# anands-repo/hello

Hardware: AMD Instinct MI355X
Metric: candidate sites/sec (whole node) (higher is better)
Workload: dtype f32

## Files before the change

### hello_amd/compiler.py

```python
from __future__ import annotations

from dataclasses import dataclass, field
from typing import Dict, List, Optional, Tuple

import numpy as np

from . import netspec as ns
from . import weights as wts

ROWS_READS0, ROWS_READS1, ROWS_ALLELES, ROWS_SITES = 0, 1, 2, 3
SEG_R0A, SEG_R1A, SEG_AS = 0, 1, 2
BUF_NONE, BUF_READS0, BUF_READS1, BUF_REF, BUF_FIRST_SCRATCH = -1, 0, 1, 2, 3
OP_XATTN_FRONT = 11
(OP_CONV1D, OP_MAXPOOL, OP_SEGSUM, OP_MIX, OP_HEAD, OP_CONCAT, OP_ADD, OP_READCONV_FUSED, OP_LAYERNORM,
 OP_COMPRESSOR_FUSED) = range(1, 11)
FLAG_RELU, FLAG_SRC_U8, FLAG_SOFTMAX, FLAG_MIX_REST, FLAG_SOFTPLUS, FLAG_WINOGRAD, FLAG_BF16X3, FLAG_BF16X3_32 = 1, 2, 4, 8, 16, 32, 64, 128
FLAG_LANE_SHIFT, MAX_LANES = 8, 8
OP_NAMES = {1: "conv1d", 2: "maxpool", 3: "segsum", 4: "mix", 5: "head", 6: "concat", 7: "add",
            8: "readconv_fused", 9: "layernorm", 10: "compressor_fused", 11: "xattn_front"}


@dataclass
class Value:
    vid: int
    domain: int
    length: int
    channels: int
    u8: bool = False

    @property
    def floats_per_row(self):
        return self.length * self.channels


@dataclass
class Op:
    kind: int
    domain: int
    src0: int = BUF_NONE
    src1: int = BUF_NONE
    dst: int = BUF_NONE
    res: int = BUF_NONE
    cin: int = 0
    cout: int = 0
    k: int = 0
    stride: int = 1
    pad: int = 0
    lin: int = 0
    lout: int = 0
# ... 498 lines not shown
        return n_experts, has_meta


def _fold_site_sums(ops: List[Op]) -> List[Op]:
    drop = set()
    for o in ops:
        if o.kind != OP_XATTN_FRONT or o.src1 == BUF_NONE:
            continue
        makers = [j for j, m in enumerate(ops) if m.kind == OP_SEGSUM and m.dst == o.src1]
        readers = [r for r in ops if r is not o and o.src1 in (r.src0, r.src1, r.res)]
        if len(makers) == 1 and not readers and ops[makers[0]].seg == SEG_AS and ops[makers[0]].src0 == o.src0:
            drop.add(makers[0])
            o.src1 = BUF_NONE
    return [o for j, o in enumerate(ops) if j not in drop]


def _fold_concats(ops: List[Op]) -> List[Op]:
    drop = set()
    for j, c in enumerate(ops):
        if c.kind != OP_CONCAT or c.cin % 16 or c.c1 % 16:
            continue
        readers = [r for r in ops if r is not c and c.dst in (r.src0, r.src1, r.res)]
        if len(readers) != 1:
            continue
        r = readers[0]
        if (r.kind == OP_CONV1D and r.src0 == c.dst and r.src1 == BUF_NONE and r.res == BUF_NONE and r.c1 <= 1
                and (r.flags & FLAG_WINOGRAD) and (r.flags & FLAG_RELU) and not (r.flags & (FLAG_BF16X3 | FLAG_SOFTPLUS))
                and r.cin == c.cin + c.c1):
            r.src0, r.src1, r.seg = c.src0, c.src1, c.cin
            drop.add(j)
    return [o for j, o in enumerate(ops) if j not in drop]


def assign_lanes(ops: List[Op], max_lanes: int = 4) -> int:
    producer: Dict[int, int] = {}
    lane_of: List[int] = []
    tail: Dict[int, int] = {}
    for i, o in enumerate(ops):
        front = o.kind == OP_XATTN_FRONT
        reads = [v for v in (o.src0, o.src1, BUF_NONE if front else o.res) if v >= 1000 and v in producer]
        pick = next((lane_of[producer[v]] for v in reads if tail.get(lane_of[producer[v]]) == producer[v]), None)
        if pick is None:
            unused = [lane for lane in range(max_lanes) if lane not in tail]
            pick = unused[0] if unused else (lane_of[producer[reads[0]]] if reads else 0)
        lane_of.append(pick)
        tail[pick] = i
        o.flags = (o.flags & ~(7 << FLAG_LANE_SHIFT)) | (pick << FLAG_LANE_SHIFT)
        if o.kind != OP_HEAD:
            producer[o.dst] = i
        if front:
            producer[o.res] = i
    return len(tail)


_SMALL_LAUNCH_US = {OP_READCONV_FUSED: 75.0, OP_COMPRESSOR_FUSED: 55.0, OP_XATTN_FRONT: 27.0, OP_CONV1D: 10.0, OP_HEAD: 8.0, OP_SEGSUM: 7.0}


def schedule_lanes(ops: List[Op]) -> List[Op]:
    shift = FLAG_LANE_SHIFT
    n = len(ops)
    producer: Dict[int, int] = {}
    preds: List[set] = [set() for _ in range(n)]
    last_on_lane: Dict[int, int] = {}
    for i, o in enumerate(ops):
        front = o.kind == OP_XATTN_FRONT
        for v in (o.src0, o.src1, BUF_NONE if front else o.res):
# ... 39 lines not shown
        if pool:
            fits = [p for p in pool if phys[p][1] >= need]
            pick = min(fits, key=lambda p: phys[p][1]) if fits else max(pool, key=lambda p: phys[p][1])
            pool.remove(pick)
            phys[pick] = (v.domain, max(phys[pick][1], need))
        else:
            pick = len(phys)
            phys.append((v.domain, need))
        assigned[vid] = pick

    for i, o in enumerate(ops):
        if o.kind == OP_XATTN_FRONT:
            place(o.dst)
            place(o.res)
            for vsrc in {o.src0, o.src1}:
                if reuse and vsrc >= 1000 and last_use.get(vsrc) == i and vsrc in assigned:
                    free[values[vsrc].domain].append(assigned[vsrc])
            continue
        if o.kind != OP_HEAD:
            place(o.dst)
        for vsrc in {o.src0, o.src1, o.res}:
            if reuse and vsrc >= 1000 and last_use.get(vsrc) == i and vsrc in assigned:
                free[values[vsrc].domain].append(assigned[vsrc])
    for o in ops:
        o.src0 = assigned.get(o.src0, o.src0)
        o.src1 = assigned.get(o.src1, o.src1)
        o.res = assigned.get(o.res, o.res)
        if o.kind != OP_HEAD:
            o.dst = assigned[o.dst]
    return phys


def compile_model(spec: ns.ModelSpec, state, fused: bool = True, winograd: bool = True, arithmetic: str = "fp32",
                  fold_site_sums: bool = True, lanes: bool = False) -> Program:
    low = _Lowering(spec, state, fused, winograd, arithmetic)
    n_experts, has_meta = low.lower()
    if arithmetic != "fp32" and not low.used_bf16x3:
        raise ValueError("arithmetic='bf16x3' / 'bf16x3+32' exists for the canonical 150 bp ReLU read convolver in the whole-kernel "
                         "Winograd form (fused=True, winograd=True): this model / these options do not run it")
    if fold_site_sums:
        low.ops = _fold_site_sums(low.ops)
        low.ops = _fold_concats(low.ops)
    n_lanes = assign_lanes(low.ops) if lanes else 1
    if n_lanes > 1:
        low.ops = schedule_lanes(low.ops)
    buffers = _allocate(low.ops, low.values, reuse=n_lanes == 1)
    return Program(
        spec_name=spec.name, window=spec.window, channels0=spec.channels[0],
        channels1=spec.channels[1] if spec.hybrid_inputs else 0,
        n_experts=n_experts, has_meta=has_meta, uses_ref=low.uses_ref, ops=low.ops,
        buffers=buffers, weights=low.blob.finish(), fused_read_convolver=low.used_fused,
        fused_compressor=low.used_fused_compressor, winograd=low.winograd, arithmetic=arithmetic, n_lanes=n_lanes)
```

### hello_amd/csrc/engine.hip

```cpp
#include <hip/hip_runtime.h>

#include <cstdarg>
#include <cstdio>
#include <cstring>
#include <new>
#include <stdexcept>
#include <string>
#include <vector>

#include "../../include/hello_mi355x.h"
#include "kernels.h"

namespace {

thread_local std::string g_last_error;

int fail(int code, const char* fmt, ...) {
    char buf[512];
    va_list ap;
    va_start(ap, fmt);
    vsnprintf(buf, sizeof(buf), fmt, ap);
    va_end(ap);
    g_last_error = buf;
    return code;
// ... 63 lines not shown
        if (bytes <= cap) return 0;
        if (p) (void)hipHostFree(p);
        p = nullptr;
        size_t want = bytes + bytes / 8 + 256;
        if (hipHostMalloc(&p, want, hipHostMallocDefault) != hipSuccess) return -1;
        cap = want;
        return 0;
    }
    void release() {
        if (p) (void)hipHostFree(p);
        p = nullptr;
        cap = 0;
    }
};

}

struct hello_engine {
    int device = 0;
    hello_model_desc desc{};
    std::vector<hello_op> ops;
    std::vector<hello_buffer> buffers;
    float* d_weights = nullptr;
    size_t n_weight_floats = 0;

    std::vector<DevBuf> scratch;
    DevBuf d_csr;
    PinnedBuf h_csr;
    DevBuf d_logits, d_meta, d_post, d_rcl0, d_rcl1;
    DevBuf d_out_small;
    PinnedBuf h_io;
    std::vector<DevBuf> d_partial;
    std::vector<int> partial_of;
    int n_lanes = 1;
    std::vector<hipStream_t> lane_streams;
    std::vector<hipEvent_t> op_done;
    std::vector<std::vector<int>> op_waits;
    std::vector<int> lane_tail;
    hipEvent_t ev_lanes_go = nullptr;
    DevBuf d_feat_in, d_feat_out;
    DevBuf d_support;
    hipStream_t own_stream = nullptr;
    hipStream_t last_stream = nullptr;
    hipEvent_t ev_staged = nullptr;
    hipEvent_t ev_start = nullptr, ev_stop = nullptr;
    bool staged_pending = false;
    bool timed = false;
    bool profiling = false;
    std::vector<std::vector<hipEvent_t>> prof_events;
    int prof_count = 0;
    int prof_filter = 0;
    int debug_op = -1;
    DevBuf d_debug;
    size_t debug_floats = 0;
    int stamp_mode = 0;
    DevBuf d_stamps;
    int32_t stamp_layout[5] = {0, 0, 0, 0, 0};

    int32_t *roff0 = nullptr, *roff1 = nullptr, *aoff = nullptr, *site_of_allele = nullptr;
    int32_t *allele_of_read0 = nullptr, *allele_of_read1 = nullptr;
    int32_t *group_slot0 = nullptr, *group_slot1 = nullptr, *slot_off0 = nullptr, *slot_off1 = nullptr;
    hello::ReadConvPlan plan0{1, 0, 0}, plan1{1, 0, 0};
    bool wide_trunk[2] = {false, false};
    int64_t* pair_off = nullptr;
};

// ... 249 lines not shown
    const int n_ops = d->n_ops;
    auto lane_of = [&](int i) { return lane_of_op(d->ops[i]); };
    for (int i = 0; i < n_ops; ++i) plan.n_lanes = lane_of(i) + 1 > plan.n_lanes ? lane_of(i) + 1 : plan.n_lanes;
    if (plan.n_lanes == 1) return 0;
    std::vector<int> writer(d->n_buffers, -1);
    plan.op_waits.assign(n_ops, {});
    plan.lane_tail.assign(plan.n_lanes, -1);
    plan.read_elsewhere.assign(n_ops, 0);
    for (int i = 0; i < n_ops; ++i) {
        const hello_op& o = d->ops[i];
        const bool front = o.kind == HELLO_OP_XATTN_FRONT;
        const int reads[3] = {o.src0, o.src1, front ? HELLO_BUF_NONE : o.res};
        for (int b : reads) {
            if (b < HELLO_BUF_FIRST_SCRATCH) continue;
            const int w = writer[b];
            if (w < 0) return fail(HELLO_ERR_MODEL, "laned program: op %d reads buffer %d before any op wrote it", i, b);
            if (lane_of(w) != lane_of(i)) {
                plan.op_waits[i].push_back(w);
                plan.read_elsewhere[w] = 1;
            }
        }
        const int writes[2] = {o.kind == HELLO_OP_HEAD ? HELLO_BUF_NONE : o.dst, front ? o.res : HELLO_BUF_NONE};
        for (int b : writes) {
            if (b < HELLO_BUF_FIRST_SCRATCH) continue;
            if (writer[b] >= 0)
                return fail(HELLO_ERR_MODEL, "laned program: ops %d and %d both write buffer %d (a program with lanes may not reuse buffers)", writer[b], i, b);
            writer[b] = i;
        }
        plan.lane_tail[lane_of(i)] = i;
    }
    return 0;
}

template <typename T>
T* carve(char*& cursor, size_t count) {
    T* p = reinterpret_cast<T*>(cursor);
    cursor += (count * sizeof(T) + 15) & ~size_t(15);
    return p;
}

}

extern "C" {

const char* hello_last_error(void) { return g_last_error.c_str(); }
int hello_abi_version(void) { return HELLO_ABI_VERSION; }

int hello_engine_create(const hello_model_desc* desc, const void* folded_weights, size_t nbytes,
                        int hip_device, hello_engine** out) try {
    if (!out) return fail(HELLO_ERR_ARG, "out is NULL");
    *out = nullptr;
    if (int rc = validate_model(desc)) return rc;
    LanePlan lanes;
    if (int rc = analyse_lanes(desc, lanes)) return rc;
    if (!folded_weights || nbytes == 0 || (nbytes % 4)) return fail(HELLO_ERR_ARG, "bad weight blob");
    int n_dev = 0;
    if (hipGetDeviceCount(&n_dev) != hipSuccess || n_dev <= 0)
        return fail(HELLO_ERR_NOGPU, "no HIP device visible: the HIP engine cannot run");
    if (hip_device < 0 || hip_device >= n_dev) return fail(HELLO_ERR_ARG, "device %d out of range", hip_device);
    hipDeviceProp_t prop;
    HIP_TRY(hipGetDeviceProperties(&prop, hip_device));
    if (strncmp(prop.gcnArchName, "gfx950", 6) != 0)
        return fail(HELLO_ERR_NOGPU, "device %d is %s; this engine is built for gfx950 only", hip_device,
                    prop.gcnArchName);
    HIP_TRY(hipSetDevice(hip_device));

    hello_engine* e = new hello_engine();
    e->device = hip_device;
    e->desc = *desc;
    e->ops.assign(desc->ops, desc->ops + desc->n_ops);
    e->buffers.assign(desc->buffers, desc->buffers + desc->n_buffers);
    e->desc.ops = e->ops.data();
    e->desc.buffers = e->buffers.data();
    e->n_weight_floats = nbytes / 4;
    for (const hello_op& o : e->ops) {
        size_t w_end = 0, b_end = 0;
        if (o.kind == HELLO_OP_CONV1D) {
            const bool wino = (o.flags & HELLO_FLAG_WINOGRAD) != 0;
            const size_t cpad = wino ? (size_t)o.cout : (size_t)((o.cout + 31) / 32) * 32;
            const int cing = o.cin / (o.c1 > 1 ? o.c1 : 1);
            const size_t kpad = wino ? (size_t)(hello::conv1d_wino_outputs_per_tile(o.lin) + 2) * cing
                                     : (size_t)((o.k * cing + 31) / 32) * 32;
            w_end = (size_t)o.w_off + cpad * kpad;
            b_end = (size_t)o.b_off + cpad;
        } else if (o.kind == HELLO_OP_HEAD) {
            w_end = (size_t)o.w_off + (size_t)o.cout * o.cin;
            b_end = (size_t)o.b_off + o.cout;
        } else if (o.kind == HELLO_OP_LAYERNORM) {
            w_end = (size_t)o.w_off + o.cin;
            b_end = (size_t)o.b_off + o.cin;
        } else if (o.kind == HELLO_OP_COMPRESSOR_FUSED) {
            w_end = (size_t)o.w_off + hello::compressor_weight_floats(o.k);
            b_end = (size_t)o.b_off;
        } else if (o.kind == HELLO_OP_XATTN_FRONT) {
            w_end = (size_t)o.w_off + hello::xattn_front_weight_floats();
            b_end = (size_t)o.b_off;
        } else if (o.kind == HELLO_OP_READCONV_FUSED) {
            w_end = (size_t)o.w_off + (o.cout == 128 ? hello::readconv_wide_weight_floats()
                                                     : hello::readconv_weight_floats(o.k, (o.flags & HELLO_FLAG_WINOGRAD) != 0, desc->window));
            b_end = (size_t)o.b_off;
            if (o.cout == 128) e->wide_trunk[o.seg == HELLO_SEG_READS1_TO_ALLELES ? 1 : 0] = true;
        }
        if (w_end > e->n_weight_floats || b_end > e->n_weight_floats) {
            delete e;
            return fail(HELLO_ERR_MODEL, "a weight block runs past the end of the blob");
        }
    }
// ... 439 lines not shown
            if (e->partial_of[i] >= 0)
                if (int rc = ensure(e->d_partial[e->partial_of[i]], slots * hello::readconv_frame_rows(d.window) * frame_ch * sizeof(float))) return rc;
    }
    if (d.n_experts == 3) HIP_TRY(hipMemsetAsync(d_logits, 0, logit_bytes, stream));

    auto ptr = [&](int id) -> void* {
        if (id == HELLO_BUF_NONE) return nullptr;
        if (id < HELLO_BUF_FIRST_SCRATCH) return const_cast<void*>(buf_ptr[id]);
        return e->scratch[id].p;
    };

    HIP_TRY(hipEventRecord(e->ev_start, stream));
    int op_index = 0;
    std::vector<hipEvent_t>* ring = nullptr;
    if (e->profiling && e->prof_count < (int)e->prof_events.size() &&
        e->prof_events[e->prof_count].size() == e->ops.size() + 1)
        ring = &e->prof_events[e->prof_count];
    auto mark = [&](int slot) -> int {
        hipEvent_t& ev = (*ring)[slot];
        if (!ev) HIP_TRY(hipEventCreate(&ev));
        HIP_TRY(hipEventRecord(ev, stream));
        return 0;
    };
    const int n_ops_total = (int)e->ops.size();
    auto wanted = [&](int i) { return i >= 0 && i < n_ops_total && (!e->prof_filter || e->ops[i].kind == e->prof_filter); };
    const bool laned = e->n_lanes > 1;
    if (laned) {
        if (ring || e->debug_op >= 0 || (e->stamp_mode & 1))
            return fail(HELLO_ERR_ARG, "per-op profiling / debug capture / stamps need the sequential program (this engine runs lanes)");
        HIP_TRY(hipEventRecord(e->ev_lanes_go, stream));
        for (int l = 1; l < e->n_lanes; ++l) HIP_TRY(hipStreamWaitEvent(e->lane_streams[l], e->ev_lanes_go, 0));
    }
    hipStream_t const call_stream = stream;
    for (const hello_op& o : e->ops) {
        const int lane = laned ? (o.flags & HELLO_FLAG_LANE_MASK) >> HELLO_FLAG_LANE_SHIFT : 0;
        hipStream_t const stream = lane ? e->lane_streams[lane] : call_stream;
        if (laned)
            for (int w : e->op_waits[op_index]) HIP_TRY(hipStreamWaitEvent(stream, e->op_done[w], 0));
        if (ring && (wanted(op_index) || wanted(op_index - 1)))
            if (int rc = mark(op_index)) return rc;
        const long long rows = rows_of(o.domain, S, A, R0, R1);
        switch (o.kind) {
            case HELLO_OP_CONV1D: {
                hello::ConvArgs a{};
                a.src = ptr(o.src0);
                a.dst = (float*)ptr(o.dst);
                a.res = (const float*)ptr(o.res);
                a.w = e->d_weights + o.w_off;
                a.bias = e->d_weights + o.b_off;
                a.m_total = rows * o.lout;
                a.groups = o.c1 > 1 ? o.c1 : 1;
                a.src2 = o.src1 != HELLO_BUF_NONE ? (const float*)ptr(o.src1) : nullptr;
                a.split = o.src1 != HELLO_BUF_NONE ? o.seg : 0;
                a.lin = o.lin; a.lout = o.lout; a.cin = o.cin / a.groups; a.cin_stride = o.cin; a.cout = o.cout;
                a.k = o.k; a.stride = o.stride; a.pad = o.pad;
                a.kpad = ((o.k * a.cin + 31) / 32) * 32;
                a.cout_pad = ((o.cout + 31) / 32) * 32;
                a.relu = (o.flags & HELLO_FLAG_RELU) ? 1 : ((o.flags & HELLO_FLAG_SOFTPLUS) ? 2 : 0);
                a.src_u8 = (o.flags & HELLO_FLAG_SRC_U8) ? 1 : 0;
                a.wino = (o.flags & HELLO_FLAG_WINOGRAD) ? 1 : 0;
                if (!a.src) return fail(HELLO_ERR_ARG, "op %d reads an input the caller did not supply", op_index);
                if (a.wino) {
                    a.kpad = (hello::conv1d_wino_outputs_per_tile(o.lin) + 2) * a.cin;
                    a.cout_pad = o.cout;
                    if (!hello::conv1d_wino_supported(a))
                        return fail(HELLO_ERR_MODEL, "op %d: this convolution has no Winograd form", op_index);
// ... 14 lines not shown
                                             o.lin * o.cin, stream));
                break;
            }
            case HELLO_OP_MIX:
                HIP_TRY(hello::launch_mix((const float*)ptr(o.src0), (const float*)ptr(o.src1), (float*)ptr(o.dst),
                                          e->site_of_allele, rows, o.lin * o.cin, o.a0, o.a1,
                                          (o.flags & HELLO_FLAG_MIX_REST) != 0, stream));
                break;
            case HELLO_OP_HEAD: {
                float* outp;
                long long so, sr;
                if (o.dst == 3) { outp = d_meta; so = 1; sr = 3; }
                else { outp = d_logits + (long long)o.dst * A; so = 0; sr = 1; }
                HIP_TRY(hello::launch_head((const float*)ptr(o.src0), e->d_weights + o.w_off, e->d_weights + o.b_off,
                                           outp, rows, o.lin, o.cin, o.cout, so, sr,
                                           (o.flags & HELLO_FLAG_SOFTMAX) ? 1 : 0, stream));
                break;
            }
            case HELLO_OP_CONCAT:
                HIP_TRY(hello::launch_concat((const float*)ptr(o.src0), (const float*)ptr(o.src1), (float*)ptr(o.dst),
                                             rows * o.lin, o.cin, o.c1, stream));
                break;
            case HELLO_OP_ADD:
                HIP_TRY(hello::launch_add((const float*)ptr(o.src0), (const float*)ptr(o.src1), (float*)ptr(o.dst),
                                          rows * o.lin * o.cin, stream));
                break;
            case HELLO_OP_COMPRESSOR_FUSED: {
                hello::CompressorArgs a{};
                a.frames = (const float*)ptr(o.src0);
                a.dst = (float*)ptr(o.dst);
                a.w = e->d_weights + o.w_off;
                a.n_items = rows;
                a.blocks = o.k;
                HIP_TRY(hello::launch_compressor_fused(a, stream));
                break;
            }
            case HELLO_OP_XATTN_FRONT: {
                hello::XattnFrontArgs a{};
                a.alleles = (const float*)ptr(o.src0);
                a.sites = o.src1 == HELLO_BUF_NONE ? nullptr : (const float*)ptr(o.src1);
                a.owner = e->site_of_allele;
                a.site_off = e->aoff;
                a.y2 = (float*)ptr(o.dst);
                a.sc = (float*)ptr(o.res);
                a.w = e->d_weights + o.w_off;
                a.n_items = rows;
                a.a0 = o.a0;
                a.a1 = o.a1;
                a.rest = (o.flags & HELLO_FLAG_MIX_REST) ? 1 : 0;
                HIP_TRY(hello::launch_xattn_front(a, stream));
                break;
            }
            case HELLO_OP_LAYERNORM:
                HIP_TRY(hello::launch_layernorm((const float*)ptr(o.src0), (const float*)ptr(o.res), (float*)ptr(o.dst),
                                                e->d_weights + o.w_off, e->d_weights + o.b_off, rows * o.lin, o.cin, o.a0,
                                                (o.flags & HELLO_FLAG_RELU) ? 1 : ((o.flags & HELLO_FLAG_SOFTPLUS) ? 2 : 0), stream));
                break;
            case HELLO_OP_READCONV_FUSED: {
                const bool t1 = o.seg == HELLO_SEG_READS1_TO_ALLELES;
                hello::ReadConvArgs a{};
                if (o.flags & HELLO_FLAG_SRC_U8) {
                    a.reads = (const uint8_t*)ptr(o.src0);
                    a.channels = o.cin;
                } else {
                    a.pooled = (const float*)ptr(o.src0);
                }
// ... 23 lines not shown
                    const int stamp_waves = hello::readconv_stamp_waves();
                    if ((e->stamp_mode & 1) && !t1 && total > 0) {
                        if (wide || !a.reads) return fail(HELLO_ERR_ARG, "stamps: the canonical fused read convolver from the bytes only");
                        const long long wgs = plan.rest_wgs ? plan.bulk_wgs + plan.rest_wgs : (long long)((total + (long long)G * plan.groups_per_wg - 1) / ((long long)G * plan.groups_per_wg));
                        const int slots = hello::readconv_stamp_slots();
                        const size_t bytes = (size_t)wgs * stamp_waves * plan.groups_per_wg * slots * sizeof(uint64_t);
                        if (bytes > e->d_stamps.cap) {
                            HIP_TRY(hipStreamSynchronize(stream));
                            if (e->d_stamps.ensure(bytes)) return fail(HELLO_ERR_HIP, "device allocation of %zu bytes failed", bytes);
                        }
                        HIP_TRY(hipMemsetAsync(e->d_stamps.p, 0, bytes, stream));
                        a.stamps = (unsigned long long*)e->d_stamps.p;
                        a.stamp_groups = plan.groups_per_wg;
                        a.stamp_mode = e->stamp_mode;
                        const int32_t lay[5] = {(int32_t)wgs, stamp_waves, plan.groups_per_wg, slots, (int32_t)(plan.rest_wgs ? plan.bulk_wgs : wgs)};
                        for (int i = 0; i < 5; ++i) stamp_lay[i] = lay[i];
                        e->stamp_layout[0] = 0;
                    }
                    HIP_TRY(wide ? hello::launch_readconv_wide(a, stream) : hello::launch_readconv_fused(a, stream));
                    if (plan.rest_wgs) {
                        hello::ReadConvArgs b = a;
                        if (b.stamps) b.stamps += (size_t)plan.bulk_wgs * stamp_waves * plan.groups_per_wg * hello::readconv_stamp_slots();
                        if (b.reads) b.reads += bulk_reads * d.window * o.cin;
                        else b.pooled += bulk_reads * (long long)o.lin * o.cin;
                        b.allele_of_read += bulk_reads;
                        b.slot_of_group += plan.bulk_wgs;
                        b.groups_per_wg = 1;
                        b.n_reads = total - bulk_reads;
                        HIP_TRY(wide ? hello::launch_readconv_wide(b, stream) : hello::launch_readconv_fused(b, stream));
                    }
                    if (a.stamps)
                        for (int i = 0; i < 5; ++i) e->stamp_layout[i] = stamp_lay[i];
                }
                HIP_TRY(hello::launch_readconv_finalize((const float*)e->d_partial[e->partial_of[op_index]].p, t1 ? e->slot_off1 : e->slot_off0,
                                                        (float*)ptr(o.dst), A, o.lout, o.cout, stream));
                break;
            }
        }
        if (op_index == e->debug_op) {
            const size_t per_row = o.kind == HELLO_OP_CONCAT ? (size_t)o.lout * (o.cin + o.c1)
                                   : (o.kind == HELLO_OP_CONV1D || o.kind == HELLO_OP_READCONV_FUSED || o.kind == HELLO_OP_COMPRESSOR_FUSED || o.kind == HELLO_OP_XATTN_FRONT) ? (size_t)o.lout * o.cout
                                   : (o.kind == HELLO_OP_MAXPOOL ? (size_t)o.lout * o.cin : (size_t)o.lin * o.cin);
            const size_t n = (size_t)rows * per_row;
            if (n * sizeof(float) > e->d_debug.cap) {
                HIP_TRY(hipStreamSynchronize(stream));
                if (e->d_debug.ensure(n * sizeof(float))) return fail(HELLO_ERR_HIP, "device allocation of %zu bytes failed", n * sizeof(float));
            }
            HIP_TRY(hipMemcpyAsync(e->d_debug.p, ptr(o.dst), n * sizeof(float), hipMemcpyDeviceToDevice, stream));
            e->debug_floats = n;
        }
        if (laned && e->op_done[op_index]) HIP_TRY(hipEventRecord(e->op_done[op_index], stream));
        ++op_index;
    }
    if (laned)
        for (int l = 1; l < e->n_lanes; ++l)
            if (e->lane_tail[l] >= 0) HIP_TRY(hipStreamWaitEvent(stream, e->op_done[e->lane_tail[l]], 0));
    if (ring) {
        if (int rc = mark(op_index)) return rc;
        e->prof_count++;
    }
    if (posteriors)
        HIP_TRY(hello::launch_posteriors(d_logits, d.n_experts == 3 ? d_meta : nullptr, e->aoff, e->pair_off, S, A,
                                         d.n_experts, n_pairs, d_post, stream));
    HIP_TRY(hipEventRecord(e->ev_stop, stream));
    e->timed = true;

    char* const h_out = out_total_small ? (char*)e->h_io.p + SMALL_IO : nullptr;
    if (out_total_small) {
// ... 227 lines not shown
```

### hello_amd/csrc/kernels.h

```cpp
#pragma once
#include <hip/hip_runtime.h>
#include <stdint.h>

namespace hello {

int device_cus();

struct ConvArgs {
    const void* src;
    const float* src2;
    int split;
    float* dst;
    const float* res;
    const float* w;
    const float* bias;
    long long m_total;
    int lin, lout, cin, cout, k, stride, pad;
    int cin_stride;
    int groups;
    int kpad;
    int cout_pad;
    int relu;
    int src_u8;
    unsigned wino_rows;
// ... 46 lines not shown
    int winograd;
    int window;
    int softplus;
    int bf16x3;
    unsigned long long* stamps;
    int stamp_groups;
    int stamp_mode;
};
int readconv_stamp_slots();
int readconv_stamp_waves();
bool readconv_supports_window(int window);
int readconv_reads_per_group(int window);
int readconv_frame_rows(int window);
int readconv_groups_per_workgroup(long long n_reads, int window);
struct ReadConvPlan {
    int groups_per_wg;
    long long bulk_wgs;
    long long rest_wgs;
};
ReadConvPlan readconv_plan(long long n_reads, int window);
ReadConvPlan readconv_wide_plan(long long n_reads);
int readconv_weight_floats(int extra_blocks, bool winograd, int window);
int readconv_bf16x3_extra_floats(int extra_blocks);
bool readconv_supports_extra_blocks(int extra_blocks);
hipError_t launch_readconv_fused(const ReadConvArgs& a, hipStream_t stream);
hipError_t launch_readconv_finalize(const float* partial, const int32_t* slot_off, float* frames, int n_alleles,
                                    int frame_rows, int channels, hipStream_t stream);
int readconv_wide_weight_floats();
int readconv_wide_reads_per_group();
hipError_t launch_readconv_wide(const ReadConvArgs& a, hipStream_t stream);

struct CompressorArgs {
    const float* frames;
    float* dst;
    const float* w;
    long long n_items;
    int blocks;
    int items_per_wg;
};
int small_launch_items_per_wg(long long n_items, int most);
int compressor_weight_floats(int blocks);
bool compressor_supports_blocks(int blocks);
hipError_t launch_compressor_fused(const CompressorArgs& a, hipStream_t stream);

struct XattnFrontArgs {
    const float* alleles;
    const float* sites;
    const int32_t* owner;
    const int32_t* site_off;
    float* y2;
    float* sc;
    const float* w;
    long long n_items;
    float a0, a1;
    int rest;
    int items_per_wg;
};
int xattn_front_weight_floats();
hipError_t launch_xattn_front(const XattnFrontArgs& a, hipStream_t stream);

struct FeaturizeArgs {
    const uint8_t* bases;
    const uint8_t* quals;
    const long long* read_off;
    const uint32_t* cigars;
    const long long* cigar_off;
// ... 28 lines not shown
```

### hello_amd/csrc/readconv_fused.hip

```cpp
#include <cstdlib>
#include <type_traits>

#include "kernels.h"

namespace hello {

typedef float f32x4 __attribute__((ext_vector_type(4)));

namespace rc {

constexpr int S1_STEPS = 6;
template <bool WINO, bool F33 = false>
struct Offs {
    static constexpr int KT = WINO ? 4 : 3;
    static constexpr int W3232 = 2 * KT * 2 * 256, W3264 = 4 * 3 * 2 * 256, W3264S = 4 * 1 * 2 * 256;
    static constexpr int W6464 = 4 * KT * 4 * 256;
    static constexpr int W6464D = F33 ? 4 * 5 * 4 * 256 : W6464;
    static constexpr int W3232D = F33 ? 2 * 5 * 2 * 256 : W3232;
    static constexpr int OFF_B = 0;
    static constexpr int OFF_C1 = OFF_B + 6 * (W3232D + 32);
    static constexpr int OFF_SC = OFF_C1 + W3264 + 64;
    static constexpr int OFF_C2 = OFF_SC + W3264S + 64;
    static constexpr int OFF_D = OFF_C2 + W6464D + 64;
    static constexpr int W_TRUNK = OFF_D + 6 * (W6464D + 64);
// ... 1567 lines not shown
    static constexpr int THREADS = 64 * NW;
    static constexpr int L0 = 36, L1 = 18;
    static constexpr int NSREG = 3 * (L1 * G / 48);
    static constexpr int BUF_FLOATS = rc::cmax((L0 * G + 2) * 64, (L1 * G + 2) * 128);
    static constexpr int LDS_BYTES = 2 * BUF_FLOATS * 4 + 64;
    static constexpr int W11 = 4 * 1 * 4 * 256, WS = 8 * 3 * 4 * 256, WSC = 8 * 1 * 4 * 256, WB = 8 * 8 * 5 * 256;
    static constexpr int OFF_11 = 0, OFF_S = OFF_11 + W11 + 64, OFF_SC = OFF_S + WS + 128, OFF_B = OFF_SC + WSC + 128;
    static constexpr int off_conv(int i) { return OFF_B + i * (WB + 128); }
    static constexpr int total(int blocks) { return off_conv(1 + 2 * blocks); }
};
}

int compressor_weight_floats(int blocks) { return cc::Cfg::total(blocks); }
bool compressor_supports_blocks(int blocks) { return blocks >= 2 && blocks <= 4; }

template <int NB>
__global__ __launch_bounds__(cc::Cfg::THREADS, 2) void compressor_kernel(CompressorArgs a) {
    using CF = cc::Cfg;
    constexpr int G = CF::G, L0 = CF::L0, L1 = CF::L1;
    extern __shared__ __attribute__((aligned(16))) float smem[];
    float* const bufA = smem;
    float* const bufB = smem + CF::BUF_FLOATS;
    float* const dump = smem + 2 * CF::BUF_FLOATS;
    const int tid = threadIdx.x, lane = tid & 63;
    const int wave = __builtin_amdgcn_readfirstlane(tid >> 6);
    const long long item0 = (long long)blockIdx.x * a.items_per_wg;
    const int n_here = (int)((a.n_items - item0) < a.items_per_wg ? (a.n_items - item0) : a.items_per_wg);
    const float* __restrict__ W = a.w;
    const f32x4 zero4 = {0.f, 0.f, 0.f, 0.f};

    f32x4 w11[4];
    load_weights<4>(w11, W + CF::OFF_11, wave % 4, lane);
    {
        const f32x4* src = (const f32x4*)(a.frames + item0 * (L0 * 64));
        constexpr int NLD = G * L0 * 16 / CF::THREADS;
        static_assert(NLD * CF::THREADS == G * L0 * 16, "the input image divides evenly over the threads");
        f32x4 v[NLD];
#pragma unroll
        for (int k = 0; k < NLD; ++k) {
            const int f = tid + CF::THREADS * k;
            v[k] = (f / (L0 * 16)) < n_here ? src[f] : zero4;
        }
#pragma unroll
        for (int k = 0; k < NLD; ++k) {
            const int f = tid + CF::THREADS * k;
            *(f32x4*)(bufA + img_off<64, SW_OLD>(1 + (f >> 4), f & 15)) = v[k];
        }
        if (tid < 16) ((f32x4*)bufA)[tid] = zero4;
        else if (tid < 32) ((f32x4*)bufB)[tid - 16] = zero4;
    }
    __syncthreads();
    f32x4 sreg[CF::NSREG];
    const bool full = n_here == G;
    const int live0 = (n_here * L0 + 15) / 16, live1 = (n_here * L1 + 15) / 16;
    if (full)
        conv_layer<CF, 64, 64, 1, 1, 0, L0, L0, L0, L0 * G / 16, MODE_PLAIN, false, GEOM_TRUNK, 16, L0 * G, false, SW_OLD, SW_W>(
            bufA, bufB, w11, nullptr, W + CF::OFF_11 + CF::W11, sreg, 0u, dump, wave, lane);
    else
        conv_layer<CF, 64, 64, 1, 1, 0, L0, L0, L0, L0 * G / 16, MODE_PLAIN, false, GEOM_TRUNK, 16, L0 * G, false, SW_OLD, SW_W, true>(
            bufA, bufB, w11, nullptr, W + CF::OFF_11 + CF::W11, sreg, 0u, dump, wave, lane, 0, (live0 - wave / 4 + 1) / 2);
    f32x4 ws[12], wsc[4];
    load_weights<12>(ws, W + CF::OFF_S, wave, lane);
    load_weights<4>(wsc, W + CF::OFF_SC, wave, lane);
    __syncthreads();
    if (tid < 64) ((f32x4*)bufA)[(tid & 31) + (tid >> 5) * (L1 * G + 1) * 32] = zero4;
    if (full)
        conv_layer<CF, 64, 128, 3, 2, 1, L0, L1, L1, L1 * G / 16, MODE_PLAIN, false, GEOM_TRUNK, 16, L1 * G, true, SW_W, SW_3>(
            bufB, bufA, ws, nullptr, W + CF::OFF_S + CF::WS, sreg, 0u, dump, wave, lane);
    else
        conv_layer<CF, 64, 128, 3, 2, 1, L0, L1, L1, L1 * G / 16, MODE_PLAIN, false, GEOM_TRUNK, 16, L1 * G, true, SW_W, SW_3, true>(
            bufB, bufA, ws, nullptr, W + CF::OFF_S + CF::WS, sreg, 0u, dump, wave, lane, 0, live1);
    conv_layer<CF, 64, 128, 1, 2, 0, L0, L1, L1, CF::NSREG, MODE_TO_REGS, false, GEOM_WTRIPLE, 16, L1 * G, false, SW_W, SW_3>(
        bufB, nullptr, wsc, nullptr, W + CF::OFF_SC + CF::WSC, sreg, 0u, dump, wave, lane);
    f32x4 w3[2][5];
// ... 16 lines not shown
        __syncthreads();
        static_for<0, NB>([&](auto bc) {
            constexpr int blk = decltype(bc)::value;
            constexpr int off_a = CF::off_conv(1 + 2 * blk), off_b = CF::off_conv(2 + 2 * blk);
            wino3_layer<CF, 128, MODE_PLAIN, false, L1, SW_3, true, PARTIAL>(bufB, bufA, w3, slice(off_a), slice(off_b),
                                                                            W + off_a + CF::WB, wave, lane, live_tiles);
            __syncthreads();
            if constexpr (blk < NB - 1)
                wino3_layer<CF, 128, MODE_RESID_INPLACE, false, L1, SW_3, true, PARTIAL>(
                    bufA, bufB, w3, slice(off_b), slice(CF::off_conv(3 + 2 * blk)), W + off_b + CF::WB, wave, lane, live_tiles);
            else
                wino3_layer<CF, 128, MODE_RESID_INPLACE, true, L1, SW_3, true, PARTIAL>(bufA, bufB, w3, slice(off_b), nullptr,
                                                                                       W + off_b + CF::WB, wave, lane, live_tiles);
            __syncthreads();
        });
    };
    if (live_tiles == L1 * G / 48) f33_layers(std::false_type{});
    else f33_layers(std::true_type{});
    f32x4* dst = (f32x4*)(a.dst + item0 * (L1 * 128));
    for (int f = tid; f < n_here * L1 * 32; f += CF::THREADS)
        dst[f] = *(const f32x4*)(bufB + img_off<128, SW_3>(1 + (f >> 5), f & 31));
}

int small_launch_items_per_wg(long long n_items, int most) {
    const long long cus = device_cus();
    const long long n = (n_items + cus - 1) / cus;
    return (int)(n < 1 ? 1 : (n <= 2 ? n : most));
}

hipError_t launch_compressor_fused(const CompressorArgs& args, hipStream_t stream) {
    if (args.n_items <= 0) return hipSuccess;
    CompressorArgs a = args;
    if (a.items_per_wg == 0) a.items_per_wg = small_launch_items_per_wg(a.n_items, cc::Cfg::G);
    if (!compressor_supports_blocks(a.blocks) || !a.frames || !a.dst || !a.w || a.items_per_wg < 1 || a.items_per_wg > cc::Cfg::G) return hipErrorInvalidValue;
    static bool configured_on[64] = {};
    int dev = 0;
    if (hipGetDevice(&dev) != hipSuccess || dev < 0 || dev >= 64) return hipErrorInvalidDevice;
    if (!configured_on[dev]) {
        hipError_t e = hipFuncSetAttribute((const void*)compressor_kernel<2>, hipFuncAttributeMaxDynamicSharedMemorySize, cc::Cfg::LDS_BYTES);
        if (e == hipSuccess)
            e = hipFuncSetAttribute((const void*)compressor_kernel<3>, hipFuncAttributeMaxDynamicSharedMemorySize, cc::Cfg::LDS_BYTES);
        if (e == hipSuccess)
            e = hipFuncSetAttribute((const void*)compressor_kernel<4>, hipFuncAttributeMaxDynamicSharedMemorySize, cc::Cfg::LDS_BYTES);
        if (e != hipSuccess) return e;
        configured_on[dev] = true;
    }
    const unsigned grid = (unsigned)((a.n_items + a.items_per_wg - 1) / a.items_per_wg);
    if (a.blocks == 2) hipLaunchKernelGGL(compressor_kernel<2>, dim3(grid), dim3(cc::Cfg::THREADS), cc::Cfg::LDS_BYTES, stream, a);
    else if (a.blocks == 3) hipLaunchKernelGGL(compressor_kernel<3>, dim3(grid), dim3(cc::Cfg::THREADS), cc::Cfg::LDS_BYTES, stream, a);
    else hipLaunchKernelGGL(compressor_kernel<4>, dim3(grid), dim3(cc::Cfg::THREADS), cc::Cfg::LDS_BYTES, stream, a);
    return hipGetLastError();
}


namespace xf {
struct Cfg {
    static constexpr int ACT = rc::ACT_RELU;
    static __device__ __forceinline__ float act(float x) { return fmaxf(x, 0.f); }
    static constexpr int G = 8, NW = 8, THREADS = 64 * NW;
    static constexpr int L = 18, LO = 9;
    static constexpr int NSREG = 1;
    static constexpr int A_FLOATS = (L * G + 2) * 128;
    static constexpr int B_ROWS = 2 * (16 * 5) + 2;
    static constexpr int LDS_BYTES = (A_FLOATS + B_ROWS * 128) * 4 + 64;
    static constexpr int W11 = 8 * 1 * 8 * 256, WS = 16 * 3 * 8 * 256, WSC = 16 * 1 * 8 * 256;
    static constexpr int OFF_11 = 0, OFF_S = OFF_11 + W11 + 128, OFF_SC = OFF_S + WS + 256, TOTAL = OFF_SC + WSC + 256;
};
// ... 492 lines not shown
```

### hello_amd/engine.py

```python
from __future__ import annotations

import ctypes as C
import logging
import os
from typing import Optional, Sequence, Tuple

import numpy as np

from . import compiler
from . import netspec as ns

_log = logging.getLogger(__name__)

_LIB_PATH = os.environ.get("HELLO_LIB") or os.path.join(os.path.dirname(os.path.abspath(__file__)),
                                                        "libhello_mi355x.so")
HELLO_IN_DEVICE, HELLO_OUT_DEVICE, HELLO_LAYOUT_RCL = 1, 2, 4
ABI_VERSION = 2
LANES_MAX_SITES = 64

class HelloOp(C.Structure):
    _fields_ = [("kind", C.c_int32), ("domain", C.c_int32), ("src0", C.c_int32), ("src1", C.c_int32),
                ("dst", C.c_int32), ("res", C.c_int32), ("cin", C.c_int32), ("cout", C.c_int32),
                ("k", C.c_int32), ("stride", C.c_int32), ("pad", C.c_int32), ("lin", C.c_int32),
                ("lout", C.c_int32), ("flags", C.c_int32), ("seg", C.c_int32), ("c1", C.c_int32),
# ... 68 lines not shown


def _is_torch(x):
    return type(x).__module__.startswith("torch")


def _i32_host(x) -> np.ndarray:
    if _is_torch(x):
        x = x.detach().cpu().numpy()
    return np.ascontiguousarray(np.asarray(x), dtype=np.int32)


def n_pairs(alleles_per_site) -> int:
    a = np.asarray(alleles_per_site, dtype=np.int64)
    return int((a * (a + 1) // 2).sum())


def model_desc(program: "compiler.Program"):
    ops = (HelloOp * len(program.ops))()
    for dst, o in zip(ops, program.ops):
        for name, _ in HelloOp._fields_:
            setattr(dst, name, getattr(o, name))
    bufs = (HelloBuffer * len(program.buffers))()
    for dst, (dom, fpr) in zip(bufs, program.buffers):
        dst.domain, dst.floats_per_row = dom, fpr
    desc = HelloModelDesc(ABI_VERSION, program.window, program.channels0, program.channels1, program.n_experts, int(program.has_meta),
                          int(program.uses_ref), len(program.buffers), bufs, len(program.ops), ops)
    return desc, (ops, bufs)


class Engine:

    def __init__(self, spec: ns.ModelSpec, state, device: int = 0, fused: bool = True, winograd: bool = True,
                 program: Optional["compiler.Program"] = None, arithmetic: Optional[str] = None, lanes_max_sites: Optional[int] = None):
        self.lib = load_library()
        self.spec = spec
        self.lanes_max_sites = lanes_max_sites
        self._lanes_recipe = None if program is not None else dict(state=state, fused=fused, winograd=winograd, arithmetic=arithmetic or "fp32")
        if program is None:
            program = compiler.compile_model(spec, state, fused=fused, winograd=winograd, arithmetic=arithmetic or "fp32")
        self.program = program
        p = self.program
        self.device = device
        self.handle, self._desc_arrays = self._create(p)
        self.lanes_handle = None
        self.lanes_program = None
        self._sequential_only = 0
        self.n_experts = p.n_experts
        self.has_meta = p.has_meta
        self._own = None

    def _create(self, program):
        desc, keep = model_desc(program)
        blob = np.ascontiguousarray(program.weights, dtype=np.float32)
        handle = C.c_void_p()
        _check(self.lib.hello_engine_create(C.byref(desc), blob.ctypes.data, blob.nbytes, self.device, C.byref(handle)))
        return handle, keep

    def small_launch_handle(self):
        if self._sequential_only or self._lanes_recipe is None:
            return self.handle
        if self.lanes_handle is None:
            r = self._lanes_recipe
            prog = compiler.compile_model(self.spec, r["state"], fused=r["fused"], winograd=r["winograd"], arithmetic=r["arithmetic"], lanes=True)
            if prog.n_lanes == 1:
                self._lanes_recipe = None
                return self.handle
            self.lanes_handle, self._lanes_desc_arrays = self._create(prog)
            self.lanes_program = prog
            self._lanes_recipe = dict(r, state=None)
        return self.lanes_handle

    class _OnStream:
# ... 230 lines not shown
```

### include/hello_mi355x.h

```cpp
#ifndef HELLO_MI355X_H
#define HELLO_MI355X_H

#include <stddef.h>
#include <stdint.h>

#ifdef __cplusplus
extern "C" {
#endif

#define HELLO_ABI_VERSION 2

typedef enum hello_status {
    HELLO_OK = 0,
    HELLO_ERR_ARG = -1,
    HELLO_ERR_SHAPE = -2,
    HELLO_ERR_MODEL = -3,
    HELLO_ERR_HIP = -4,
    HELLO_ERR_NOGPU = -5,
    HELLO_ERR_NOMEM = -6
} hello_status;


typedef enum hello_domain {
    HELLO_ROWS_READS0 = 0,
// ... 12 lines not shown
#define HELLO_BUF_READS0 0
#define HELLO_BUF_READS1 1
#define HELLO_BUF_REF    2
#define HELLO_BUF_FIRST_SCRATCH 3

typedef enum hello_op_kind {
    HELLO_OP_CONV1D = 1,
    HELLO_OP_MAXPOOL = 2,
    HELLO_OP_SEGSUM = 3,
    HELLO_OP_MIX = 4,
    HELLO_OP_HEAD = 5,
    HELLO_OP_CONCAT = 6,
    HELLO_OP_ADD = 7,
    HELLO_OP_READCONV_FUSED = 8
    ,
    HELLO_OP_LAYERNORM = 9
    ,
    HELLO_OP_COMPRESSOR_FUSED = 10
    ,
    HELLO_OP_XATTN_FRONT = 11
} hello_op_kind;

#define HELLO_FLAG_RELU     1
#define HELLO_FLAG_SRC_U8   2
#define HELLO_FLAG_SOFTMAX  4
#define HELLO_FLAG_SOFTPLUS 16
#define HELLO_FLAG_WINOGRAD 32
#define HELLO_FLAG_BF16X3   64
#define HELLO_FLAG_BF16X3_32 128
#define HELLO_FLAG_MIX_REST 8
#define HELLO_FLAG_LANE_SHIFT 8
#define HELLO_FLAG_LANE_MASK  (7 << HELLO_FLAG_LANE_SHIFT)
#define HELLO_MAX_LANES 8

typedef struct hello_op {
    int32_t kind;
    int32_t domain;
    int32_t src0, src1;
    int32_t dst;
    int32_t res;
    int32_t cin, cout;
    int32_t k, stride, pad;
    int32_t lin, lout;
    int32_t flags;
    int32_t seg;
    int32_t c1;
    float a0, a1;
    int64_t w_off;
    int64_t b_off;
} hello_op;

typedef struct hello_buffer {
    int32_t domain;
    int32_t floats_per_row;
} hello_buffer;

typedef struct hello_model_desc {
    int32_t abi_version;
    int32_t window;
    int32_t channels0, channels1;
    int32_t n_experts;
    int32_t has_meta;
    int32_t uses_ref;
    int32_t n_buffers;
    const hello_buffer* buffers;
    int32_t n_ops;
// ... 248 lines not shown
```

Before: 484,800.

## Fold read-convolver finalize into fused compressor by reading partial slots directly

Adds a compiler pass and an engine analysis that mark a fused compressor whose only input comes from a fused read convolver with [36][64] frames. The separate finalize kernel, which sums per-read partial slots into frames, is then skipped, and the compressor sums the slot rows itself while loading its input. This removes one kernel launch and a full write and read of the intermediate frame buffer. In exchange the compressor's load loop gains data-dependent iteration counts and scattered slot reads, which can be uneven across threads.

```diff
diff --git a/hello_amd/compiler.py b/hello_amd/compiler.py
--- a/hello_amd/compiler.py
+++ b/hello_amd/compiler.py
@@ -15,6 +15,7 @@
 (OP_CONV1D, OP_MAXPOOL, OP_SEGSUM, OP_MIX, OP_HEAD, OP_CONCAT, OP_ADD, OP_READCONV_FUSED, OP_LAYERNORM,
  OP_COMPRESSOR_FUSED) = range(1, 11)
 FLAG_RELU, FLAG_SRC_U8, FLAG_SOFTMAX, FLAG_MIX_REST, FLAG_SOFTPLUS, FLAG_WINOGRAD, FLAG_BF16X3, FLAG_BF16X3_32 = 1, 2, 4, 8, 16, 32, 64, 128
+FLAG_FROM_SLOTS = 2048
 FLAG_LANE_SHIFT, MAX_LANES = 8, 8
 OP_NAMES = {1: "conv1d", 2: "maxpool", 3: "segsum", 4: "mix", 5: "head", 6: "concat", 7: "add",
             8: "readconv_fused", 9: "layernorm", 10: "compressor_fused", 11: "xattn_front"}
@@ -579,6 +580,25 @@
     return [o for j, o in enumerate(ops) if j not in drop]
 
 
+def _fold_finalize(ops: List[Op]) -> List[Op]:
+    if sum(o.kind == OP_READCONV_FUSED for o in ops) != 1:
+        return ops
+    for i, c in enumerate(ops):
+        if c.kind != OP_COMPRESSOR_FUSED:
+            continue
+        makers = [j for j, m in enumerate(ops) if m.kind != OP_HEAD and m.dst == c.src0]
+        readers = [r for r in ops if r is not c and c.src0 in (r.src0, r.src1, r.res)]
+        if len(makers) != 1 or readers or makers[0] > i:
+            continue
+        m = ops[makers[0]]
+        if m.kind != OP_READCONV_FUSED or (m.lout, m.cout) != (36, 64):
+            continue
+        if any(o.kind == OP_READCONV_FUSED and o.seg == m.seg for o in ops[makers[0] + 1:i]):
+            continue
+        c.flags |= FLAG_FROM_SLOTS
+    return ops
+
+
 def assign_lanes(ops: List[Op], max_lanes: int = 4) -> int:
     producer: Dict[int, int] = {}
     lane_of: List[int] = []
@@ -684,7 +704,7 @@
 
 
 def compile_model(spec: ns.ModelSpec, state, fused: bool = True, winograd: bool = True, arithmetic: str = "fp32",
-                  fold_site_sums: bool = True, lanes: bool = False) -> Program:
+                  fold_site_sums: bool = True, lanes: bool = False, fold_finalize: bool = True) -> Program:
     low = _Lowering(spec, state, fused, winograd, arithmetic)
     n_experts, has_meta = low.lower()
     if arithmetic != "fp32" and not low.used_bf16x3:
@@ -693,6 +713,8 @@
     if fold_site_sums:
         low.ops = _fold_site_sums(low.ops)
         low.ops = _fold_concats(low.ops)
+    if fold_finalize and not lanes:
+        low.ops = _fold_finalize(low.ops)
     n_lanes = assign_lanes(low.ops) if lanes else 1
     if n_lanes > 1:
         low.ops = schedule_lanes(low.ops)
diff --git a/hello_amd/csrc/engine.hip b/hello_amd/csrc/engine.hip
--- a/hello_amd/csrc/engine.hip
+++ b/hello_amd/csrc/engine.hip
@@ -119,6 +119,8 @@
     PinnedBuf h_io;
     std::vector<DevBuf> d_partial;
     std::vector<int> partial_of;
+    std::vector<int> slots_from;
+    std::vector<int> slots_into;
     int n_lanes = 1;
     std::vector<hipStream_t> lane_streams;
     std::vector<hipEvent_t> op_done;
@@ -434,6 +436,37 @@
     return 0;
 }
 
+int analyse_slot_folds(const hello_model_desc* d, int n_lanes, std::vector<int>& slots_from, std::vector<int>& slots_into) {
+    slots_from.assign(d->n_ops, -1);
+    slots_into.assign(d->n_ops, -1);
+    auto writes = [&](const hello_op& o, int b) {
+        return (o.kind != HELLO_OP_HEAD && o.dst == b) || (o.kind == HELLO_OP_XATTN_FRONT && o.res == b);
+    };
+    auto reads = [&](const hello_op& o, int b) {
+        return o.src0 == b || o.src1 == b || (o.kind != HELLO_OP_XATTN_FRONT && o.res == b);
+    };
+    for (int i = 0; i < d->n_ops; ++i) {
+        const hello_op& c = d->ops[i];
+        if (!(c.flags & HELLO_FLAG_FROM_SLOTS)) continue;
+        if (c.kind != HELLO_OP_COMPRESSOR_FUSED)
+            return fail(HELLO_ERR_MODEL, "op %d (%s): HELLO_FLAG_FROM_SLOTS belongs to a fused compressor", i, op_name(c.kind));
+        if (n_lanes > 1) return fail(HELLO_ERR_MODEL, "op %d: HELLO_FLAG_FROM_SLOTS is for the sequential program (this one runs lanes)", i);
+        int m = i - 1;
+        while (m >= 0 && !writes(d->ops[m], c.src0)) --m;
+        if (m < 0 || d->ops[m].kind != HELLO_OP_READCONV_FUSED || d->ops[m].cout != 64 || d->ops[m].lout != 36)
+            return fail(HELLO_ERR_MODEL, "op %d: HELLO_FLAG_FROM_SLOTS needs src0 written by a fused read convolver with [36][64] frames", i);
+        for (int j = m + 1; j < i; ++j)
+            if (d->ops[j].kind == HELLO_OP_READCONV_FUSED && d->ops[j].seg == d->ops[m].seg)
+                return fail(HELLO_ERR_MODEL, "op %d: HELLO_FLAG_FROM_SLOTS, but op %d rewrites the partial slots of op %d before they are read", i, j, m);
+        for (int j = m + 1; j < d->n_ops && (j == m + 1 || !writes(d->ops[j - 1], c.src0)); ++j)
+            if (j != i && reads(d->ops[j], c.src0))
+                return fail(HELLO_ERR_MODEL, "op %d: HELLO_FLAG_FROM_SLOTS, but op %d reads the frames of op %d too", i, j, m);
+        slots_from[i] = m;
+        slots_into[m] = i;
+    }
+    return 0;
+}
+
 template <typename T>
 T* carve(char*& cursor, size_t count) {
     T* p = reinterpret_cast<T*>(cursor);
@@ -455,6 +488,8 @@
     if (int rc = validate_model(desc)) return rc;
     LanePlan lanes;
     if (int rc = analyse_lanes(desc, lanes)) return rc;
+    std::vector<int> slots_from, slots_into;
+    if (int rc = analyse_slot_folds(desc, lanes.n_lanes, slots_from, slots_into)) return rc;
     if (!folded_weights || nbytes == 0 || (nbytes % 4)) return fail(HELLO_ERR_ARG, "bad weight blob");
     int n_dev = 0;
     if (hipGetDeviceCount(&n_dev) != hipSuccess || n_dev <= 0)
@@ -475,6 +510,8 @@
     e->desc.ops = e->ops.data();
     e->desc.buffers = e->buffers.data();
     e->n_weight_floats = nbytes / 4;
+    e->slots_from = std::move(slots_from);
+    e->slots_into = std::move(slots_into);
     for (const hello_op& o : e->ops) {
         size_t w_end = 0, b_end = 0;
         if (o.kind == HELLO_OP_CONV1D) {
@@ -980,6 +1017,7 @@
         for (int l = 1; l < e->n_lanes; ++l) HIP_TRY(hipStreamWaitEvent(e->lane_streams[l], e->ev_lanes_go, 0));
     }
     hipStream_t const call_stream = stream;
+    auto stays_in_slots = [&](int readconv) { return readconv >= 0 && e->slots_into[readconv] >= 0 && e->debug_op != readconv; };
     for (const hello_op& o : e->ops) {
         const int lane = laned ? (o.flags & HELLO_FLAG_LANE_MASK) >> HELLO_FLAG_LANE_SHIFT : 0;
         hipStream_t const stream = lane ? e->lane_streams[lane] : call_stream;
@@ -1060,6 +1098,11 @@
                 a.w = e->d_weights + o.w_off;
                 a.n_items = rows;
                 a.blocks = o.k;
+                if (stays_in_slots(e->slots_from[op_index])) {
+                    const int maker = e->slots_from[op_index];
+                    a.partial = (const float*)e->d_partial[e->partial_of[maker]].p;
+                    a.slot_off = e->ops[maker].seg == HELLO_SEG_READS1_TO_ALLELES ? e->slot_off1 : e->slot_off0;
+                }
                 HIP_TRY(hello::launch_compressor_fused(a, stream));
                 break;
             }
@@ -1149,8 +1192,9 @@
                     if (a.stamps)
                         for (int i = 0; i < 5; ++i) e->stamp_layout[i] = stamp_lay[i];
                 }
-                HIP_TRY(hello::launch_readconv_finalize((const float*)e->d_partial[e->partial_of[op_index]].p, t1 ? e->slot_off1 : e->slot_off0,
-                                                        (float*)ptr(o.dst), A, o.lout, o.cout, stream));
+                if (!stays_in_slots(op_index))
+                    HIP_TRY(hello::launch_readconv_finalize((const float*)e->d_partial[e->partial_of[op_index]].p, t1 ? e->slot_off1 : e->slot_off0,
+                                                            (float*)ptr(o.dst), A, o.lout, o.cout, stream));
                 break;
             }
         }
diff --git a/hello_amd/csrc/kernels.h b/hello_amd/csrc/kernels.h
--- a/hello_amd/csrc/kernels.h
+++ b/hello_amd/csrc/kernels.h
@@ -102,6 +102,8 @@
 
 struct CompressorArgs {
     const float* frames;
+    const float* partial;
+    const int32_t* slot_off;
     float* dst;
     const float* w;
     long long n_items;
diff --git a/hello_amd/csrc/readconv_fused.hip b/hello_amd/csrc/readconv_fused.hip
--- a/hello_amd/csrc/readconv_fused.hip
+++ b/hello_amd/csrc/readconv_fused.hip
@@ -1623,14 +1623,42 @@
     f32x4 w11[4];
     load_weights<4>(w11, W + CF::OFF_11, wave % 4, lane);
     {
-        const f32x4* src = (const f32x4*)(a.frames + item0 * (L0 * 64));
         constexpr int NLD = G * L0 * 16 / CF::THREADS;
         static_assert(NLD * CF::THREADS == G * L0 * 16, "the input image divides evenly over the threads");
         f32x4 v[NLD];
-#pragma unroll
-        for (int k = 0; k < NLD; ++k) {
-            const int f = tid + CF::THREADS * k;
-            v[k] = (f / (L0 * 16)) < n_here ? src[f] : zero4;
+        if (!a.partial) {
+            const f32x4* src = (const f32x4*)(a.frames + item0 * (L0 * 64));
+#pragma unroll
+            for (int k = 0; k < NLD; ++k) {
+                const int f = tid + CF::THREADS * k;
+                v[k] = (f / (L0 * 16)) < n_here ? src[f] : zero4;
+            }
+        } else {
+            const f32x4* first[NLD];
+            int count[NLD], most = 0;
+#pragma unroll
+            for (int k = 0; k < NLD; ++k) {
+                const int f = tid + CF::THREADS * k;
+                const int it = f / (L0 * 16);
+                count[k] = 0;
+                first[k] = (const f32x4*)a.partial;
+                v[k] = zero4;
+                if (it < n_here) {
+                    const int lo = a.slot_off[item0 + it];
+                    count[k] = a.slot_off[item0 + it + 1] - lo;
+                    first[k] = (const f32x4*)a.partial + (long long)lo * (L0 * 16) + (f - it * (L0 * 16));
+                    if (count[k] > 0) v[k] = first[k][0];
+                    most = count[k] > most ? count[k] : most;
+                }
+            }
+            for (int r = 1; r < most; ++r) {
+                f32x4 row[NLD];
+#pragma unroll
+                for (int k = 0; k < NLD; ++k) row[k] = r < count[k] ? first[k][(long long)r * (L0 * 16)] : zero4;
+#pragma unroll
+                for (int k = 0; k < NLD; ++k)
+                    if (r < count[k]) v[k] = v[k] + row[k];
+            }
         }
 #pragma unroll
         for (int k = 0; k < NLD; ++k) {
@@ -1713,7 +1741,8 @@
     if (args.n_items <= 0) return hipSuccess;
     CompressorArgs a = args;
     if (a.items_per_wg == 0) a.items_per_wg = small_launch_items_per_wg(a.n_items, cc::Cfg::G);
-    if (!compressor_supports_blocks(a.blocks) || !a.frames || !a.dst || !a.w || a.items_per_wg < 1 || a.items_per_wg > cc::Cfg::G) return hipErrorInvalidValue;
+    if (!compressor_supports_blocks(a.blocks) || !a.dst || !a.w || a.items_per_wg < 1 || a.items_per_wg > cc::Cfg::G) return hipErrorInvalidValue;
+    if ((a.partial != nullptr) != (a.slot_off != nullptr) || (!a.partial && !a.frames)) return hipErrorInvalidValue;
     static bool configured_on[64] = {};
     int dev = 0;
     if (hipGetDevice(&dev) != hipSuccess || dev < 0 || dev >= 64) return hipErrorInvalidDevice;
diff --git a/hello_amd/engine.py b/hello_amd/engine.py
--- a/hello_amd/engine.py
+++ b/hello_amd/engine.py
@@ -124,13 +124,15 @@
 class Engine:
 
     def __init__(self, spec: ns.ModelSpec, state, device: int = 0, fused: bool = True, winograd: bool = True,
-                 program: Optional["compiler.Program"] = None, arithmetic: Optional[str] = None, lanes_max_sites: Optional[int] = None):
+                 program: Optional["compiler.Program"] = None, arithmetic: Optional[str] = None, lanes_max_sites: Optional[int] = None,
+                 fold_finalize: bool = True):
         self.lib = load_library()
         self.spec = spec
         self.lanes_max_sites = lanes_max_sites
         self._lanes_recipe = None if program is not None else dict(state=state, fused=fused, winograd=winograd, arithmetic=arithmetic or "fp32")
         if program is None:
-            program = compiler.compile_model(spec, state, fused=fused, winograd=winograd, arithmetic=arithmetic or "fp32")
+            program = compiler.compile_model(spec, state, fused=fused, winograd=winograd, arithmetic=arithmetic or "fp32",
+                                             fold_finalize=fold_finalize)
         self.program = program
         p = self.program
         self.device = device
diff --git a/include/hello_mi355x.h b/include/hello_mi355x.h
--- a/include/hello_mi355x.h
+++ b/include/hello_mi355x.h
@@ -68,6 +68,7 @@
 #define HELLO_FLAG_LANE_SHIFT 8
 #define HELLO_FLAG_LANE_MASK  (7 << HELLO_FLAG_LANE_SHIFT)
 #define HELLO_MAX_LANES 8
+#define HELLO_FLAG_FROM_SLOTS 2048
 
 typedef struct hello_op {
     int32_t kind;
```

Result: no change. 485,700, median of 6 (+0.2%).
